# stresearch/xfr

Measured on AMD Instinct MI355X. Metric: triplet-contrastive-EBP saliency maps/sec, ResNet-101 224x224, higher is better.
Workload: dtype f32

## Files before the change

xfr_amd/csrc/conv_gemm.hip:

```cpp
#include <algorithm>
#include <atomic>
#include <mutex>
#include <vector>
#include "common.h"
#include <cstdio>
#include <cstdlib>

#include "conv_gemm_dev.h"
#include "conv_gemm_host.h"

std::atomic<long> g_conv_chain_launches[2];

namespace {

#ifndef XFR_MFM_WAVES
#define XFR_MFM_WAVES 6
#endif
#ifndef XFR_DUAL_WAVES
#define XFR_DUAL_WAVES 4
#endif
template <int TCO, int TM, int BK, int NST, int MODE, bool RELU, int CHAIN>
__global__ __launch_bounds__(NT, CHAIN == 0 ? 1 : (CHAIN == 1 ? 7 : (CHAIN == 4 ? XFR_DUAL_WAVES : XFR_MFM_WAVES))) void conv_gemm_kernel(const ConvParams p, const int n_co_tiles, const int n_m_tiles)
{
    constexpr bool ROW = TCO == 32;
// ... 722 lines not shown
        bool same = true;
        for (int i = 0; i < XFR_MAX_EW_STEPS && same; ++i) same = kChainSigs[sgi][i] == (i < n ? codes[i] : 0);
        if (same) return sgi;
    }
    return -1;
}
int conv_gemm_num_chain_sigs() { return kNumChainSigs; }

int conv_gemm_cannot_launch(const ConvParams& p)
{
    if (p.chain.n <= 0) return 0;
    ConvParams q = p;
    return plan_chain(q);
}
const char* conv_gemm_refusal(int why)
{
    switch (why) {
        case 0: return "the convolution launch was refused without a reason";
        case 1: return "a dual (W / relu(W)) convolution launch carries a fused chain without a compiled epilogue";
        case 3: return "lean probe-forward steps and the dual-accumulator launch (ConvParams::dualacc) only exist together, behind a compiled epilogue";
        case 2: return "a fused chain with a MaxFeatureMap step (pair maximum / fan-out VJP) has no compiled epilogue and the interpreter does not run those steps";
        default: return "unknown convolution launch refusal";
    }
}

void conv_gemm_chain_launch_counts(long* compiled, long* interpreted)
{
    if (compiled) *compiled = g_conv_chain_launches[0].load();
    if (interpreted) *interpreted = g_conv_chain_launches[1].load();
}

static int pick_cfg_impl(const ConvParams& p_in, bool allow_split)
{
    ConvParams p = p_in;
    if (p.dualacc) { p.nhalves = 2; p.dualacc = 0; const int c = pick_cfg_impl(p, false); return c == CFG_ROW32 ? CFG_K16 : c; }
    if (allow_split && p.split_ok && conv_gemm_split_wanted(p)) return CFG_BF16X6;
    {
        const int rem = p.CoutTot % 64;
#ifndef XFR_NO_ROW_TILE
        if (rem > 0 && rem <= 32 && p.tap_major != 2 && p.out_stride == 1 && p.CoutTot > 32 && p.M > 64) return CFG_ROW32;
#endif
    }
    if (ks_ok<8>(p)) {
        if (p.kh == 1 && (p.stride == 2 || p.out_stride == 2 || p.as_strided)) return CFG_KS_4_4;
        if ((p.kh > 1 && p.K >= 2048) || (p.kh == 1 && (p.K == 512 || p.K >= 2048))) return CFG_KS_4_4;
    }
    const long tiles = (long)((p.CoutTot + 63) / 64) * p.nhalves * ((p.M + 63) / 64);
    if (p.K >= 1024 && tiles <= 512 && (p.tap_major ? (p.Cin % 32 == 0) : true)) return CFG_K32;
    return CFG_K16;
}
int conv_gemm_pick_cfg(const ConvParams& p_in) { return pick_cfg_impl(p_in, true); }

namespace {
struct LogRec { void* stream; int cout, nhalves, K, M, kh, chain, cfg; };
std::mutex g_tune_mu;
std::atomic<int> g_tuning{0};
unsigned long long* g_stamps = nullptr;
int g_stamps_cap = 0;
int g_stamp_regions = 0, g_stamp_seq = 0;
unsigned long long* g_log = nullptr;
int g_log_cap = 0;
std::vector<LogRec> g_log_recs;
thread_local int g_last_cfg = 0;
constexpr size_t NO_LOG = (size_t)-1;

size_t tune_begin(ConvParams& p, hipStream_t s)
{
    p.stamps = nullptr;
    p.stamps_cap = 0;
    p.stamp_regions = 0;
    p.stamp_seq = 0;
    p.span = nullptr;
    size_t log_idx = NO_LOG;
    if (g_tuning.load(std::memory_order_relaxed)) {
        std::lock_guard<std::mutex> lk(g_tune_mu);
        p.stamps = g_stamps;
        p.stamps_cap = g_stamps_cap;
        p.stamp_regions = g_stamp_regions;
        p.stamp_seq = g_stamps ? g_stamp_seq++ : 0;
        if (g_log && (int)g_log_recs.size() < g_log_cap) {
            p.span = g_log + 8 * g_log_recs.size();
            log_idx = g_log_recs.size();
            g_log_recs.push_back(LogRec{(void*)s, p.CoutTot, p.dualacc ? 2 : p.nhalves, p.K, p.M, p.kh, p.chain.n, -1});
        }
    }
    return log_idx;
}
void tune_ran(size_t log_idx, int cfg)
{
    g_last_cfg = cfg;
    if (log_idx == NO_LOG) return;
    std::lock_guard<std::mutex> lk(g_tune_mu);
    if (log_idx < g_log_recs.size()) g_log_recs[log_idx].cfg = cfg;
}
int cfg_remap(int cfg)
{
    struct Remap { int v[32]; };
    static const Remap remap = [] {
        Remap r;
        for (int i = 0; i < 32; ++i) r.v[i] = i;
        if (const char* e = getenv("XFR_CFG_REMAP")) {
            int a = 0, b = 0, n = 0;
            while (sscanf(e, "%d:%d%n", &a, &b, &n) == 2) {
                if (a >= 0 && a < 32 && b >= 0 && b < 32) r.v[a] = b;
                e += n;
                if (*e == ',') ++e;
            }
        }
        return r;
    }();
    return (cfg >= 0 && cfg < 32) ? remap.v[cfg] : cfg;
}
}

void conv_gemm_set_stamps(unsigned long long* dev_ptr, int capacity_workgroups)
{
    std::lock_guard<std::mutex> lk(g_tune_mu);
    g_stamps = dev_ptr;
    g_stamps_cap = dev_ptr ? (capacity_workgroups < 0 ? -capacity_workgroups : capacity_workgroups) : 0;
    g_stamp_regions = (dev_ptr && capacity_workgroups < 0) ? (-capacity_workgroups) / 256 : 0;
    g_stamp_seq = 0;
    g_tuning.store((g_stamps || g_log) ? 1 : 0);
}

void conv_gemm_set_log(unsigned long long* log_dev, int capacity)
{
    std::lock_guard<std::mutex> lk(g_tune_mu);
    g_log = log_dev;
    g_log_cap = log_dev ? capacity : 0;
    g_log_recs.clear();
    g_tuning.store((g_stamps || g_log) ? 1 : 0);
}
int conv_gemm_dump_log(const char* path)
{
    std::lock_guard<std::mutex> lk(g_tune_mu);
    if (!g_log) return 0;
    const size_t n = g_log_recs.size();
    std::vector<unsigned long long> h(8 * n + 8);
    if (n && hipMemcpy(h.data(), g_log, 8 * n * sizeof(unsigned long long), hipMemcpyDeviceToHost) != hipSuccess) return -1;
    FILE* f = fopen(path, "w");
    if (!f) return -1;
    fprintf(f, "seq,stream,Cout,nhalves,K,M,kh,chain,cfg,start_10ns,end_10ns\n");
    for (size_t i = 0; i < n; ++i) {
        const LogRec& r = g_log_recs[i];
        fprintf(f, "%zu,%p,%d,%d,%d,%d,%d,%d,%d,%llu,%llu\n", i, r.stream, r.cout, r.nhalves, r.K, r.M, r.kh, r.chain, r.cfg, h[8 * i], *std::max_element(h.begin() + 8 * i + 1, h.begin() + 8 * i + 8));
    }
    fclose(f);
    return (int)n;
}
int conv_gemm_last_cfg() { return g_last_cfg; }

bool launch_conv_gemm(const ConvParams& p_in, hipStream_t s)
{
    ConvParams p = p_in;
    const size_t log_idx = tune_begin(p, s);
    int cfg = p.force_cfg > 0 ? p.force_cfg : cfg_remap(conv_gemm_pick_cfg(p));
    auto ran = [&](int eff, bool ok) { tune_ran(log_idx, eff); return ok; };
    if (cfg == CFG_BF16X6) {
        if (conv_gemm_launch_split(p, s)) return ran(CFG_BF16X6, true);
        cfg = pick_cfg_impl(p, false);
    }
    if (cfg == CFG_KS_8_3 && ks_ok<8>(p)) return ran(CFG_KS_8_3, launch_cfg_ks<8, 3>(p, s));
    if (cfg == CFG_KS_4_4 && ks_ok<4>(p)) return ran(CFG_KS_4_4, launch_cfg_ks<4, 4>(p, s));
    if (cfg == CFG_K32) return ran(CFG_K32, launch_cfg<64, 64, 32, 3>(p, s));
    if (cfg == CFG_ROW32) return ran(CFG_ROW32, launch_cfg<32, 128, 16, 3>(p, s));
    return ran(CFG_K16, launch_cfg<64, 64, 16, 3>(p, s));
}
```

xfr_amd/csrc/conv_gemm_host.h:

```cpp
#pragma once
#include <atomic>
#include "common.h"

extern std::atomic<long> g_conv_chain_launches[2];
int conv_gemm_num_cus();
int conv_gemm_plan_chain(ConvParams& q);
void conv_gemm_warn_interpreted(const ConvParams& q);
bool conv_gemm_launch_split(const ConvParams& p, hipStream_t s);
bool conv_gemm_split_wanted(const ConvParams& p);
```

xfr_amd/csrc/conv_gemm_split.hip:

```cpp
#include <algorithm>
#include <atomic>
#include <mutex>
#include <unordered_map>
#include <cstdio>
#include <cstdlib>
#include <type_traits>
#include "conv_gemm_dev.h"
#include "conv_gemm_host.h"

namespace {

typedef __bf16 v8bf __attribute__((ext_vector_type(8)));
typedef unsigned v4u __attribute__((ext_vector_type(4)));
constexpr int SP_T = 128, SP_BK = 16;
constexpr int SP_A_BYTES = 3 * 2 * SP_T * 16, SP_B_BYTES = 3 * 2 * SP_T * 16;
constexpr size_t SP_LDS = 3 * (size_t)(SP_A_BYTES + SP_B_BYTES);

typedef float v2f_t __attribute__((ext_vector_type(2)));
typedef __bf16 v2bf_t __attribute__((ext_vector_type(2)));
__device__ __forceinline__ unsigned cvt_pk_bf16(float lo, float hi)
{
    const v2f_t t = {lo, hi};
    return __builtin_bit_cast(unsigned, __builtin_convertvector(t, v2bf_t));
}
__device__ __forceinline__ void split_pair(float a, float b, unsigned& p0, unsigned& p1, unsigned& p2)
{
    p0 = cvt_pk_bf16(a, b);
    const float ra = a - __uint_as_float(p0 << 16), rb = b - __uint_as_float(p0 & 0xffff0000u);
    p1 = cvt_pk_bf16(ra, rb);
    const float sa = ra - __uint_as_float(p1 << 16), sb = rb - __uint_as_float(p1 & 0xffff0000u);
    p2 = cvt_pk_bf16(sa, sb);
}

constexpr int SPP_MAX_HALO = 64, SPP_MAX_TAPS = 25;

__host__ __device__ inline int spp_halo(const ConvParams& p) { return p.pad * p.W + p.pad; }
__host__ __device__ inline int spp_patch_len(const ConvParams& p) { return SP_T + 2 * spp_halo(p); }
inline size_t spp_lds_bytes(const ConvParams& p) { return (size_t)3 * SP_A_BYTES + (size_t)2 * 6 * (spp_patch_len(p) + 1) * 16; }

constexpr int NT8 = 512;

template <int N>
__device__ __forceinline__ void sp8_wait_barrier()
{
    asm volatile("s_waitcnt vmcnt(%0) lgkmcnt(0)\n\ts_barrier" ::"n"(N) : "memory");
}

template <bool RELU, int CHAIN, bool PATCH>
__global__ __launch_bounds__(NT8, 2) void conv_gemm_split_kernel(const ConvParams p, const uint16_t* __restrict__ ws0, const uint16_t* __restrict__ ws1,
                                                                  const int n_co_tiles, const int n_m_tiles)
{
    extern __shared__ __attribute__((aligned(16))) float smem[];
    unsigned char* lds = reinterpret_cast<unsigned char*>(smem);
    constexpr int NST = 3, D = NST - 1, XBASE = NST * SP_A_BYTES;
    const int tid = threadIdx.x, lane = tid & 63, wave8 = __builtin_amdgcn_readfirstlane(tid >> 6);
    const int wr4 = wave8 >> 1, wc = wave8 & 1;
    const int l31 = lane & 31, lhi = lane >> 5;
    const bool two_dma = wave8 < 4;
    if (wave8 < 4) stamp(p, wave8, lane, 0, 4);

    const int lid = xcd_remap(blockIdx.x, n_co_tiles * n_m_tiles);
    const int tile_m = lid / n_co_tiles;
    const int tile_co_all = lid - tile_m * n_co_tiles;
    const int n_co_half = n_co_tiles / p.nhalves;
    const int half = tile_co_all / n_co_half;
    const int tile_co = tile_co_all - half * n_co_half;
    const int co0 = tile_co * SP_T, m0 = tile_m * SP_T;
    const uint16_t* __restrict__ wsel = half ? ws1 : ws0;
    const float* __restrict__ bsel = half ? p.bias_pos : p.bias;
    float* __restrict__ osel = half ? p.out1 : p.out0;
    const int T = p.kh * p.kw, ncb = p.Cin / SP_BK, nk = p.K / SP_BK;
    const int halo = spp_halo(p), PL = spp_patch_len(p);
    const int PS = PATCH ? (PL + 1) * 16 : SP_T * 16;
    const int XB = 6 * PS;
    const unsigned chan_bytes = (unsigned)p.in_nb * p.H * p.W * 4u;
    const __amdgpu_buffer_rsrc_t rW = __builtin_amdgcn_make_buffer_rsrc((void*)wsel, 0, n_co_half * nk * SP_A_BYTES, 0x00020000);
    const __amdgpu_buffer_rsrc_t rIn = __builtin_amdgcn_make_buffer_rsrc((void*)p.in, 0, (int)p.in_bytes, 0x00020000);
    const unsigned lds_base = (unsigned)(size_t)(__attribute__((address_space(3))) unsigned char*)(lds);

    unsigned t_voff = OOB, t_lds = 0;
    bool t_ok = false;
    int base_m = 0;
    unsigned long long tapmask = 0ull;
    const int sm = tid & 127, skq = wave8 >> 1;
    if constexpr (PATCH) {
        const int kh_ = tid >= PL ? 1 : 0, q = tid - kh_ * PL;
        const long g = (long)m0 - halo + q;
        t_ok = tid < 2 * PL;
        const bool in_row = t_ok && g >= 0 && g < (long)p.in_nb * p.H * p.W;
        t_voff = in_row ? (unsigned)g * 4u + (unsigned)(kh_ * 8) * chan_bytes : OOB;
        t_lds = lds_base + XBASE + kh_ * PS + q * 16;
    } else {
        const int m = m0 + sm;
        const bool m_ok = m < p.M;
        const int mm = m_ok ? m : 0;
        const int ohw = p.OH * p.OW;
        const int n = mm / ohw;
        const int r = mm - n * ohw;
        const int oh = r / p.OW;
        const int ow = r - oh * p.OW;
        const int ih0 = oh * p.stride - p.pad, iw0 = ow * p.stride - p.pad - p.pad_dw;
        base_m = n * p.H * p.W + ih0 * p.W + iw0;
        if (m_ok) {
            unsigned long long vw = 0ull;
            for (int dw = 0; dw < p.kw; ++dw)
                if ((unsigned)(iw0 + dw) < (unsigned)p.W) vw |= 1ull << dw;
            for (int dh = 0; dh < p.kh; ++dh)
                if ((unsigned)(ih0 + dh) < (unsigned)p.H) tapmask |= vw << (dh * p.kw);
        }
        t_lds = lds_base + XBASE + ((skq >> 1) * SP_T + sm) * 16 + (skq & 1) * 8;
    }
    int c_pos[2] = {0, 0};
    unsigned c_mask[2] = {0u, 0u};
    if constexpr (PATCH) {
#pragma unroll
        for (int j = 0; j < 2; ++j) {
            const int c = wc * 64 + j * 32 + l31, m = m0 + c;
            c_pos[j] = c + halo;
            unsigned mk = 0u;
            if (m < p.M) {
                const int ohw = p.OH * p.OW;
                const int r = m % ohw;
                const int oh = r / p.OW, ow = r - oh * p.OW;
                for (int dh = 0; dh < p.kh; ++dh)
                    for (int dw = 0; dw < p.kw; ++dw)
                        if ((unsigned)(oh + dh - p.pad) < (unsigned)p.H && (unsigned)(ow + dw - p.pad) < (unsigned)p.W) mk |= 1u << (dh * p.kw + dw);
            }
            c_mask[j] = mk;
        }
    }
    const unsigned char* a_lane = lds + (lhi * SP_T + wr4 * 32 + l31) * 16;
    const unsigned char* b_plane = lds + XBASE + lhi * PS;

    v16f acc[2], pipe[2];
#pragma unroll
    for (int j = 0; j < 2; ++j)
#pragma unroll
        for (int r = 0; r < 16; ++r) { acc[j][r] = 0.f; pipe[j][r] = 0.f; }

    auto dma = [&](int kt, int stage, int ch) {
        __builtin_amdgcn_raw_ptr_buffer_load_lds(rW, (lptr_t)(lds + stage * SP_A_BYTES + ch * 1024), 16, (ch * 1024 + lane * 16) | (kt < nk ? 0u : OOB),
                                                 (tile_co * nk + kt) * SP_A_BYTES, 0, 0);
    };
    auto load_w = [&](int kt, int stage) {
        dma(kt, stage, wave8);
        if (two_dma) dma(kt, stage, 8 + wave8);
    };
    auto fold = [&](bool negated) {
        if (negated) { acc[0] -= pipe[0]; acc[1] -= pipe[1]; }
        else { acc[0] += pipe[0]; acc[1] += pipe[1]; }
    };
    auto mfmas = [&](const v8bf (&af)[3], const v8bf (&bf)[3][2], auto FIRST) {
        constexpr int TA[6] = {2, 1, 0, 1, 0, 0}, TB[6] = {0, 1, 2, 0, 1, 0};
        v16f zero;
#pragma unroll
        for (int r = 0; r < 16; ++r) zero[r] = 0.f;
#pragma unroll
        for (int t = 0; t < 6; ++t)
#pragma unroll
            for (int j = 0; j < 2; ++j)
                pipe[j] = __builtin_amdgcn_mfma_f32_32x32x16_bf16(af[TA[t]], bf[TB[t]][j], (t == 0 && decltype(FIRST)::value) ? zero : pipe[j], 0, 0, 0);
    };
    std::integral_constant<int, 0> S0; std::integral_constant<int, 1> S1; std::integral_constant<int, 2> S2;
    std::integral_constant<bool, true> first; std::integral_constant<bool, false> later;

    if constexpr (PATCH) {
        float xp[8];
        auto load_patch = [&](int cb) {
            const unsigned so = (unsigned)(cb * SP_BK) * chan_bytes;
#pragma unroll
            for (int i = 0; i < 8; ++i) xp[i] = __uint_as_float(__builtin_amdgcn_raw_buffer_load_b32(rIn, t_voff, so + (unsigned)i * chan_bytes, 0));
        };
        auto store_patch = [&](int buf, unsigned flip) {
            v4u q0, q1, q2;
#pragma unroll
            for (int i = 0; i < 4; ++i) {
                const float a = RELU ? fmaxf(xp[2 * i], 0.f) : xp[2 * i], b = RELU ? fmaxf(xp[2 * i + 1], 0.f) : xp[2 * i + 1];
                unsigned h0, h1, h2;
                split_pair(a, b, h0, h1, h2);
                q0[i] = h0 ^ flip; q1[i] = h1 ^ flip; q2[i] = h2 ^ flip;
            }
            if (t_ok) {
                const unsigned at = t_lds + buf * XB;
                asm volatile("ds_write_b128 %0, %1" :: "v"(at), "v"(q0));
                asm volatile("ds_write_b128 %0, %1" :: "v"(at + 2 * PS), "v"(q1));
                asm volatile("ds_write_b128 %0, %1" :: "v"(at + 4 * PS), "v"(q2));
            }
        };
        int tap = 0, cb = 0, buf = 0, shift = -halo, tdw = 0;
        bool xl_prev = false, xl_now = false;
        const bool mfma_first = wave8 < 4;
        auto load_part = [&](int kt, v8bf (&af)[3], v8bf (&bf)[3][2]) {
            const int st1 = (kt + 1) % 3, st3 = kt % 3;
            const bool more = cb + 1 < ncb;
            xl_now = false;
            if (more && tap == 2) store_patch(buf ^ 1, ((cb + 1) & 1) ? 0x80008000u : 0u);
            load_w(kt + 3, kt < 0 ? 2 : st3);
            if (more && tap == 0) { load_patch(cb + 1); xl_now = true; }
            const unsigned char* As = a_lane + (kt < 0 ? 0 : st1) * SP_A_BYTES;
#pragma unroll
            for (int pc = 0; pc < 3; ++pc) af[pc] = *(const v8bf*)(As + pc * 2 * SP_T * 16);
#pragma unroll
            for (int j = 0; j < 2; ++j) {
                const int pos = ((c_mask[j] >> tap) & 1u) ? c_pos[j] + shift : PL;
                const unsigned char* Bs = b_plane + buf * XB + pos * 16;
#pragma unroll
                for (int pc = 0; pc < 3; ++pc) bf[pc][j] = *(const v8bf*)(Bs + pc * 2 * PS);
            }
            tap += 1; tdw += 1; shift += 1;
            if (tdw == p.kw) { tdw = 0; shift += p.W - p.kw; }
            if (tap == T) { tap = 0; shift = -halo; cb += 1; buf ^= 1; }
        };
        auto end_step = [&]() {
            if (xl_now || xl_prev) { if (two_dma) sp8_wait_barrier<10>(); else sp8_wait_barrier<9>(); }
            else { if (two_dma) sp8_wait_barrier<2>(); else sp8_wait_barrier<1>(); }
            xl_prev = xl_now;
        };
        auto step = [&](int kt, v8bf (&caf)[3], v8bf (&cbf)[3][2], v8bf (&naf)[3], v8bf (&nbf)[3][2], auto FIRST) {
            if (mfma_first) mfmas(caf, cbf, FIRST);
            __builtin_amdgcn_sched_barrier(0);
            load_part(kt, naf, nbf);
            __builtin_amdgcn_sched_barrier(0);
            if (!mfma_first) mfmas(caf, cbf, FIRST);
            end_step();
        };
        if (tid < 12) {
            const v4u z = {0u, 0u, 0u, 0u};
            asm volatile("ds_write_b128 %0, %1" :: "v"(lds_base + XBASE + (tid / 6) * XB + (tid % 6) * PS + PL * 16), "v"(z));
        }
        load_w(0, 0);
        load_w(1, 1);
        load_patch(0);
        asm volatile("s_waitcnt vmcnt(0)" ::: "memory");
        store_patch(0, 0u);
        sp8_wait_barrier<0>();
        v8bf f0a[3], f0b[3][2], f1a[3], f1b[3][2];
        load_part(-1, f0a, f0b);
        end_step();
        if (wave8 < 4) stamp(p, wave8, lane, 1);
        int pass_in_blk = 0;
        bool neg = false;
        const int passes_per_blk = T / 3;
        auto pass_done = [&]() {
            fold(neg);
            if (++pass_in_blk == passes_per_blk) { pass_in_blk = 0; neg = !neg; }
        };
        for (int kt = 0; kt < nk; kt += 6) {
            step(kt, f0a, f0b, f1a, f1b, first);
            step(kt + 1, f1a, f1b, f0a, f0b, later);
            step(kt + 2, f0a, f0b, f1a, f1b, later);
            pass_done();
            step(kt + 3, f1a, f1b, f0a, f0b, first);
            step(kt + 4, f0a, f0b, f1a, f1b, later);
            step(kt + 5, f1a, f1b, f0a, f0b, later);
            pass_done();
        }
    } else {
        int ld_tap = 0, ld_ci0 = 0;
        unsigned ld_voff = (tapmask & 1ull) ? (unsigned)base_m * 4u : OOB;
        auto load_x = [&](int kt, float (&v)[4]) {
            const unsigned voff = ld_voff | (kt < nk ? 0u : OOB);
            const unsigned so = (unsigned)(ld_ci0 + skq * 4) * chan_bytes;
#pragma unroll
            for (int i = 0; i < 4; ++i) v[i] = __uint_as_float(__builtin_amdgcn_raw_buffer_load_b32(rIn, voff, so + (unsigned)i * chan_bytes, 0));
            ld_ci0 += SP_BK;
            if (ld_ci0 >= p.Cin) {
                ld_ci0 = 0;
                ld_tap += 1;
                const int dh = ld_tap / p.kw, dw = ld_tap - dh * p.kw;
                ld_voff = (ld_tap < p.kh * p.kw && ((tapmask >> ld_tap) & 1ull)) ? (unsigned)(base_m + dh * p.W + dw) * 4u : OOB;
            }
        };
        auto store_x = [&](const float (&v)[4], int stage, unsigned flip) {
            typedef unsigned v2u __attribute__((ext_vector_type(2)));
            v2u q0, q1, q2;
#pragma unroll
            for (int i = 0; i < 2; ++i) {
                const float a = RELU ? fmaxf(v[2 * i], 0.f) : v[2 * i], b = RELU ? fmaxf(v[2 * i + 1], 0.f) : v[2 * i + 1];
                unsigned h0, h1, h2;
                split_pair(a, b, h0, h1, h2);
                q0[i] = h0 ^ flip; q1[i] = h1 ^ flip; q2[i] = h2 ^ flip;
            }
            const unsigned at = t_lds + stage * XB;
            asm volatile("ds_write_b64 %0, %1" :: "v"(at), "v"(q0));
            asm volatile("ds_write_b64 %0, %1" :: "v"(at + 2 * PS), "v"(q1));
            asm volatile("ds_write_b64 %0, %1" :: "v"(at + 4 * PS), "v"(q2));
        };
        int wst = 0;
        auto step = [&](int kt, auto ST, float (&xcur)[4], float (&xnew)[4], unsigned flip, auto FIRST) {
            constexpr int st = decltype(ST)::value, st1 = (st + 1) % 3;
            const int stD = wst + D >= NST ? wst + D - NST : wst + D;
            load_w(kt + D, stD);
            load_x(kt + 3, xnew);
            const unsigned char* As = a_lane + wst * SP_A_BYTES;
            const unsigned char* Bs = b_plane + st * XB + (wc * 64 + l31) * 16;
            v8bf af[3], bf[3][2];
#pragma unroll
            for (int pc = 0; pc < 3; ++pc) {
                af[pc] = *(const v8bf*)(As + pc * 2 * SP_T * 16);
#pragma unroll
                for (int j = 0; j < 2; ++j) bf[pc][j] = *(const v8bf*)(Bs + pc * 2 * PS + j * 32 * 16);
            }
            mfmas(af, bf, FIRST);
            store_x(xcur, st1, flip);
            if (two_dma) sp8_wait_barrier<8 + 2 * (D - 1)>(); else sp8_wait_barrier<8 + (D - 1)>();
            wst = wst + 1 == NST ? 0 : wst + 1;
        };
        float x0[4], x1[4], x2[4];
        load_w(0, 0);
        load_x(0, x0);
        asm volatile("s_waitcnt vmcnt(0)" ::: "memory");
        store_x(x0, 0, 0u);
#pragma unroll
        for (int d = 1; d < D; ++d) load_w(d, d);
        load_x(1, x0);
        load_x(2, x1);
        if (two_dma) sp8_wait_barrier<8 + 2 * (D - 1)>(); else sp8_wait_barrier<8 + (D - 1)>();
        if (wave8 < 4) stamp(p, wave8, lane, 1);
        unsigned flip = 0u;
        for (int kt = 0; kt < nk; kt += 3) {
            const bool negated = flip != 0u;
            step(kt, S0, x0, x2, flip, first);
            step(kt + 1, S1, x1, x0, flip, later);
            flip ^= 0x80008000u;
            step(kt + 2, S2, x2, x1, flip, later);
            fold(negated);
        }
    }
    wait_vmcnt<0>();
    asm volatile("s_waitcnt lgkmcnt(0)" ::: "memory");
    if (wave8 < 4) { stamp(p, wave8, lane, 2); stamp(p, wave8, lane, 3); }

#pragma unroll 1
    for (int c = 0; c < 2; ++c) {
        v16f t = acc[0];
        const int wq = (wr4 & 1) * 2 + c;
        block_epilogue<CHAIN>(p, t, smem + (wave8 - wq) * (32 * 36), tid & 255, lane, wq, co0 + (wr4 >> 1) * 64, m0 + wc * 64, half, -1, 0, 1, osel, bsel, nullptr);
        acc[0] = acc[1];
    }
    if (wave8 < 4) stamp(p, wave8, lane, 4);
}

__global__ void split_pack_kernel(const float* __restrict__ w, uint16_t* __restrict__ planes, int K, int cout, int ldw, int taps)
{
    const long idx = (long)blockIdx.x * blockDim.x + threadIdx.x;
    if (idx >= (long)K * cout) return;
    const int k = (int)(idx / cout), co = (int)(idx - (long)k * cout);
    unsigned h[3];
    split_pair(w[(long)k * ldw + co], 0.f, h[0], h[1], h[2]);
    const int cin = K / taps, tap = k / cin, ci = k - tap * cin;
    const int rt = co / SP_T, r = co - rt * SP_T, kt = (ci / SP_BK) * taps + tap, kk = ci % SP_BK, nk = K / SP_BK;
#pragma unroll
    for (int q = 0; q < 3; ++q)
        planes[((((long)(rt * nk + kt) * 3 + q) * 2 + kk / 8) * SP_T + r) * 8 + kk % 8] = (uint16_t)(h[q] & 0xffffu);
}

struct SplitPack { uint16_t* planes; int K, cout, ldw, taps; };
static std::mutex g_split_mu;
static std::unordered_map<const float*, SplitPack> g_split;

bool split_can_run(const ConvParams& p)
{
    if (p.dualacc || p.out_stride != 1 || p.as_strided || p.co_pair > 0 || p.stride != 1) return false;
    if ((p.Cin % SP_BK) != 0 || (p.K % SP_BK) != 0 || (p.CoutTot % SP_T) != 0) return false;
    if (p.kh == 1 && p.kw == 1) return p.pad == 0;
    return p.tap_major == 1 && p.kh * p.kw <= 64;
}
struct SplitPolicy { int min_k1, min_k3, min_tiles; };
const SplitPolicy& split_policy()
{
    static const SplitPolicy pol = [] {
        SplitPolicy q{256, 1152, 128};
        if (const char* e = getenv("XFR_SPLIT_MIN_K1")) q.min_k1 = atoi(e);
        if (const char* e = getenv("XFR_SPLIT_MIN_K3")) q.min_k3 = atoi(e);
        if (const char* e = getenv("XFR_SPLIT_MIN_TILES")) q.min_tiles = atoi(e);
        return q;
    }();
    return pol;
}
bool split_layer_ok(const ConvParams& p)
{
    if (!split_can_run(p)) return false;
    if (p.OH * p.OW < 196) return false;
    return p.K >= (p.kh == 1 && p.kw == 1 ? split_policy().min_k1 : split_policy().min_k3);
}
bool split_grid_ok(const ConvParams& p)
{
    const long tiles = (long)(p.CoutTot / SP_T) * p.nhalves * ((p.M + SP_T - 1) / SP_T);
    return tiles >= split_policy().min_tiles;
}

static std::atomic<long> g_split_launches{0};

bool split_patch_ok(const ConvParams& p)
{
    const int T = p.kh * p.kw;
    if (T < 5 || T > SPP_MAX_TAPS || (T % 3) != 0 || p.stride != 1 || p.tap_major != 1) return false;
    if (p.OH != p.H || p.OW != p.W || 2 * p.pad != p.kh - 1 || 2 * p.pad != p.kw - 1 || p.pad_dw != 0) return false;
    static const bool off = getenv("XFR_SPLIT_NO_PATCH") != nullptr;
    return spp_halo(p) <= SPP_MAX_HALO && !off;
}

const uint16_t* split_planes(const float* w, int K, int cout, int ldw, int taps, hipStream_t s)
{
    std::lock_guard<std::mutex> lk(g_split_mu);
    auto it = g_split.find(w);
    if (it != g_split.end())
        return (it->second.K == K && it->second.cout == cout && it->second.ldw == ldw && it->second.taps == taps) ? it->second.planes : nullptr;
    SplitPack sp{nullptr, K, cout, ldw, taps};
    if (hipMalloc(&sp.planes, (size_t)K * cout * 3 * sizeof(uint16_t)) != hipSuccess) {
        (void)hipGetLastError();
        sp.planes = nullptr;
        g_split[w] = sp;
        return nullptr;
    }
    const long n = (long)K * cout;
    hipLaunchKernelGGL(split_pack_kernel, dim3((unsigned)((n + 255) / 256)), dim3(256), 0, s, w, sp.planes, K, cout, ldw, taps);
    if (hipStreamSynchronize(s) != hipSuccess) { (void)hipFree(sp.planes); return nullptr; }
    g_split[w] = sp;
    return sp.planes;
}

template <bool RELU, int CHAIN>
void launch_split_inst(const ConvParams& q, const uint16_t* w0, const uint16_t* w1, int n_co, int n_m, hipStream_t s, bool patch)
{
    static std::atomic<unsigned long long> done{0ull};
    int dev = 0;
    (void)hipGetDevice(&dev);
    const unsigned long long bit = 1ull << (dev & 63);
    constexpr int PATCH_LDS_MAX = 3 * SP_A_BYTES + 2 * 6 * (SP_T + 2 * SPP_MAX_HALO + 1) * 16;
    if (!(done.load(std::memory_order_relaxed) & bit)) {
        (void)hipFuncSetAttribute((const void*)conv_gemm_split_kernel<RELU, CHAIN, false>, hipFuncAttributeMaxDynamicSharedMemorySize, (int)SP_LDS);
        (void)hipFuncSetAttribute((const void*)conv_gemm_split_kernel<RELU, CHAIN, true>, hipFuncAttributeMaxDynamicSharedMemorySize, PATCH_LDS_MAX);
        done.fetch_or(bit);
    }
    const dim3 grid(n_co * n_m);
    if (patch) hipLaunchKernelGGL((conv_gemm_split_kernel<RELU, CHAIN, true>), grid, dim3(NT8), spp_lds_bytes(q), s, q, w0, w1, n_co, n_m);
    else hipLaunchKernelGGL((conv_gemm_split_kernel<RELU, CHAIN, false>), grid, dim3(NT8), SP_LDS, s, q, w0, w1, n_co, n_m);
}

bool launch_split(const ConvParams& p, hipStream_t s)
{
    if (p.force_cfg == CFG_BF16X6 ? !split_can_run(p) : !conv_gemm_split_wanted(p)) return false;
    if (p.chain.n > 0 && p.relu_in) return false;
    ConvParams q = p;
    q.tail_q = 0;
    q.tail_s = 1;
    int family = p.relu_in ? -1 : 0;
    if (q.chain.n > 0) {
        if (conv_gemm_plan_chain(q)) return false;
        if (q.chain_sig >= 0 && chain_sig_is_dual(q.chain_sig)) return false;
        family = q.chain_sig < 0 ? 2 : (chain_sig_is_mfm(q.chain_sig) ? 3 : 1);
    }
    const bool patch = split_patch_ok(p);
    const int taps = patch ? p.kh * p.kw : 1;
    const uint16_t* w0 = split_planes(p.w, p.K, p.CoutTot, p.ldw, taps, s);
    const uint16_t* w1 = p.nhalves == 2 ? split_planes(p.w_pos, p.K, p.CoutTot, p.ldw, taps, s) : nullptr;
    if (!w0 || (p.nhalves == 2 && !w1)) return false;
    g_split_launches++;
    if (q.chain.n > 0) {
        g_conv_chain_launches[q.chain_sig >= 0 ? 0 : 1]++;
        if (q.chain_sig < 0) conv_gemm_warn_interpreted(q);
    }
    const int n_co = (p.CoutTot / SP_T) * p.nhalves;
    const int n_m = (p.M + SP_T - 1) / SP_T;
    switch (family) {
        case -1: launch_split_inst<true, 0>(q, w0, w1, n_co, n_m, s, patch); break;
        case 0: launch_split_inst<false, 0>(q, w0, w1, n_co, n_m, s, patch); break;
        case 1: launch_split_inst<false, 1>(q, w0, w1, n_co, n_m, s, patch); break;
        case 2: launch_split_inst<false, 2>(q, w0, w1, n_co, n_m, s, patch); break;
        default: launch_split_inst<false, 3>(q, w0, w1, n_co, n_m, s, patch); break;
    }
    return true;
}

}

void conv_gemm_forget_split(const void* lo, size_t bytes)
{
    std::lock_guard<std::mutex> lk(g_split_mu);
    const char* a = static_cast<const char*>(lo);
    for (auto it = g_split.begin(); it != g_split.end();) {
        const char* w = reinterpret_cast<const char*>(it->first);
        if (w >= a && w < a + bytes) {
            if (it->second.planes) (void)hipFree(it->second.planes);
            it = g_split.erase(it);
        } else ++it;
    }
}
int conv_gemm_split_covers(const ConvParams& p) { return split_layer_ok(p) ? 1 : 0; }
bool conv_gemm_presplit(const ConvParams& p, const float* w, hipStream_t s) { return split_planes(w, p.K, p.CoutTot, p.ldw, split_patch_ok(p) ? p.kh * p.kw : 1, s) != nullptr; }
bool conv_gemm_split_wanted(const ConvParams& p) { return split_layer_ok(p) && (p.split_ok == 2 || split_grid_ok(p)); }
bool conv_gemm_launch_split(const ConvParams& p, hipStream_t s) { return launch_split(p, s); }
long conv_gemm_split_launches() { return g_split_launches.load(); }
```

xfr_amd/csrc/engine.hip:

```cpp
#include "engine_internal.h"

namespace xfr {

thread_local std::string g_err;

xfr_status fail(xfr_status st, const char* fmt, ...)
{
    char buf[1024];
    va_list ap;
    va_start(ap, fmt);
    vsnprintf(buf, sizeof(buf), fmt, ap);
    va_end(ap);
    g_err = buf;
    return st;
}

static xfr_status allocate(xfr_engine* e)
{
    xfr_status st = layout_arena(e);
    if (st != XFR_OK) return st;
    HIP_TRY(hipMalloc(&e->arena, e->arena_floats * sizeof(float)));
    st = layout_workspace(e);
    if (st != XFR_OK) return st;
    const size_t B = (size_t)e->max_batch;
// ... 824 lines not shown
{
    if (!e || !n_firings) return fail(XFR_INVALID_ARG, "null argument");
    *n_firings = e->last_trace_firings;
    return XFR_OK;
}

xfr_status xfr_engine_get_trace(xfr_engine* e, double* sums, int32_t* kinds, int32_t capacity)
{
    if (!e || !sums) return fail(XFR_INVALID_ARG, "null argument");
    const int nf = e->last_trace_firings, SB = e->last_trace_sb;
    if (capacity < nf * SB) return fail(XFR_INVALID_ARG, "trace needs %d doubles", nf * SB);
    HIP_TRY(hipSetDevice(e->device));
    HIP_TRY(hipDeviceSynchronize());
    HIP_TRY(hipMemcpy(sums, e->dbl_ws + 2 * e->max_batch, sizeof(double) * (size_t)nf * SB, hipMemcpyDeviceToHost));
    if (kinds) for (int i = 0; i < nf; ++i) kinds[i] = e->last_trace_kinds[i];
    return XFR_OK;
}

xfr_status xfr_debug_conv(const float* in_dev, const float* w_host, const float* bias_host, float* out_dev, int32_t cin, int32_t h,
                          int32_t w, int32_t nb, int32_t cout, int32_t kh, int32_t kw, int32_t stride, int32_t pad, int32_t relu_in,
                          int32_t cfg, int32_t reps, float* ms_out)
{
    if (!in_dev || !w_host || !out_dev || cin < 1 || cout < 1 || kh < 1 || kw < 1 || stride < 1 || reps < 1)
        return fail(XFR_INVALID_ARG, "xfr_debug_conv: bad arguments");
    const int khw = kh * kw, K = cin * khw;
    const int ldw = (int)align_up(cout, 128);
    const bool tap = khw > 1 && (cin % 16 == 0) && khw <= 64;
    const bool tap4 = khw > 1 && (cin == 3 || cin == 4) && khw <= 60;
    const int Kf = tap4 ? 4 * khw : K;
    std::vector<float> host(align_up(Kf, 32) * (size_t)ldw, 0.f);
    for (int co = 0; co < cout; ++co)
        for (int ci = 0; ci < cin; ++ci)
            for (int tp = 0; tp < khw; ++tp) {
                const size_t kk = tap4 ? (size_t)tp * 4 + ci : (tap ? (size_t)tp * cin + ci : (size_t)ci * khw + tp);
                host[kk * ldw + co] = w_host[((size_t)co * cin + ci) * khw + tp];
            }
    float *wd = nullptr, *bd = nullptr;
    HIP_TRY(hipMalloc(&wd, host.size() * sizeof(float)));
    HIP_TRY(hipMemcpy(wd, host.data(), host.size() * sizeof(float), hipMemcpyHostToDevice));
    if (bias_host) {
        HIP_TRY(hipMalloc(&bd, cout * sizeof(float)));
        HIP_TRY(hipMemcpy(bd, bias_host, cout * sizeof(float), hipMemcpyHostToDevice));
    }
    ConvParams p;
    memset(&p, 0, sizeof(p));
    p.in = in_dev; p.w = wd; p.bias = bd; p.out0 = out_dev;
    p.Cin = cin; p.H = h; p.W = w; p.NB = nb; p.in_nb = nb; p.out_nb = nb;
    p.kh = kh; p.kw = kw; p.stride = stride; p.pad = pad;
    p.OH = (h + 2 * pad - kh) / stride + 1; p.OW = (w + 2 * pad - kw) / stride + 1;
    p.K = Kf; p.K_logical = K; p.M = nb * p.OH * p.OW; p.CoutTot = cout; p.nhalves = 1; p.ldw = ldw;
    p.relu_in = relu_in; p.out_H = p.OH; p.out_W = p.OW; p.out_stride = 1;
    p.in_bytes = (unsigned)((size_t)cin * nb * h * w * sizeof(float));
    p.tap_major = tap4 ? 2 : (tap ? 1 : 0); p.force_cfg = cfg % 100;
    float* tws = nullptr;
    HIP_TRY(hipMalloc(&tws, XFR_TAIL_WS_BYTES + XFR_TAIL_MAX_TILES * sizeof(unsigned)));
    p.tail_ws = tws; p.tail_ws_bytes = XFR_TAIL_WS_BYTES;
    p.tail_cnt = reinterpret_cast<unsigned*>(reinterpret_cast<char*>(tws) + XFR_TAIL_WS_BYTES);
    HIP_TRY(hipMemset(p.tail_cnt, 0, XFR_TAIL_MAX_TILES * sizeof(unsigned)));
    p.tail_force = (cfg / 10000) % 100;
    const bool split = (cfg % 100) == CFG_BF16X6;
    hipEvent_t a, b;
    HIP_TRY(hipEventCreate(&a));
    HIP_TRY(hipEventCreate(&b));
    const int nstreams = std::max(1, std::min(4, cfg / 1000000));
    p.tail_force = (cfg / 10000) % 100;
    for (int r = 0; r < std::max(1, std::min(reps, 200)); ++r) launch_conv_gemm(p, 0);
    float ms = 0.f;
    if (nstreams == 1) {
        HIP_TRY(hipEventRecord(a, 0));
        for (int r = 0; r < reps; ++r) launch_conv_gemm(p, 0);
        HIP_TRY(hipEventRecord(b, 0));
        HIP_TRY(hipDeviceSynchronize());
        HIP_TRY(hipEventElapsedTime(&ms, a, b));
    } else {
        hipStream_t st[4];
        float* tw[4];
        ConvParams q[4];
        for (int i = 0; i < nstreams; ++i) {
            HIP_TRY(hipStreamCreateWithFlags(&st[i], hipStreamNonBlocking));
            HIP_TRY(hipMalloc(&tw[i], XFR_TAIL_WS_BYTES + XFR_TAIL_MAX_TILES * sizeof(unsigned)));
            q[i] = p;
            q[i].tail_ws = tw[i];
            q[i].tail_cnt = reinterpret_cast<unsigned*>(reinterpret_cast<char*>(tw[i]) + XFR_TAIL_WS_BYTES);
            HIP_TRY(hipMemset(q[i].tail_cnt, 0, XFR_TAIL_MAX_TILES * sizeof(unsigned)));
        }
        HIP_TRY(hipDeviceSynchronize());
        HIP_TRY(hipEventRecord(a, 0));
        for (int i = 0; i < nstreams; ++i) HIP_TRY(hipStreamWaitEvent(st[i], a, 0));
        for (int r = 0; r < reps; ++r)
            for (int i = 0; i < nstreams; ++i) launch_conv_gemm(q[i], st[i]);
        for (int i = 0; i < nstreams; ++i) {
            hipEvent_t e;
            HIP_TRY(hipEventCreateWithFlags(&e, hipEventDisableTiming));
            HIP_TRY(hipEventRecord(e, st[i]));
            HIP_TRY(hipStreamWaitEvent(0, e, 0));
            (void)hipEventDestroy(e);
        }
        HIP_TRY(hipEventRecord(b, 0));
        HIP_TRY(hipDeviceSynchronize());
        HIP_TRY(hipEventElapsedTime(&ms, a, b));
        ms /= nstreams;
        for (int i = 0; i < nstreams; ++i) { (void)hipStreamDestroy(st[i]); (void)hipFree(tw[i]); }
    }
    if (ms_out) *ms_out = ms / reps;
    (void)hipEventDestroy(a); (void)hipEventDestroy(b);
    if (split) conv_gemm_forget_split(wd, host.size() * sizeof(float));
    (void)hipFree(wd);
    (void)hipFree(tws);
    if (bd) (void)hipFree(bd);
    HIP_TRY(hipGetLastError());
    return XFR_OK;
}

xfr_status xfr_debug_conv_stamps(void* stamps_dev, int32_t capacity_workgroups)
{
    if (stamps_dev && (capacity_workgroups == 0 || (capacity_workgroups < 0 && -capacity_workgroups < 256)))
        return fail(XFR_INVALID_ARG, "xfr_debug_conv_stamps: capacity must be positive (or <= -256: sampled mode)");
    conv_gemm_set_stamps(reinterpret_cast<unsigned long long*>(stamps_dev), capacity_workgroups);
    return XFR_OK;
}

xfr_status xfr_debug_conv_log(void* log_dev, int32_t capacity, const char* dump_path)
{
    if (dump_path) {
        const int n = conv_gemm_dump_log(dump_path);
        if (n < 0) return fail(XFR_HIP_ERROR, "xfr_debug_conv_log: cannot write %s", dump_path);
    }
    conv_gemm_set_log(reinterpret_cast<unsigned long long*>(log_dev), capacity);
    return XFR_OK;
}

xfr_status xfr_engine_profile_csv(xfr_engine* e, const char* path)
{
    if (!e) return fail(XFR_INVALID_ARG, "null engine");
    e->profile_csv = path ? path : "";
    return XFR_OK;
}

xfr_status xfr_chain_epilogue_stats(int64_t* compiled_launches, int64_t* interpreted_launches, int32_t* n_signatures)
{
    long c = 0, i = 0;
    conv_gemm_chain_launch_counts(&c, &i);
    if (compiled_launches) *compiled_launches = c;
    if (interpreted_launches) *interpreted_launches = i;
    if (n_signatures) *n_signatures = conv_gemm_num_chain_sigs();
    return XFR_OK;
}

xfr_status xfr_engine_memory(xfr_engine* e, size_t* weight_bytes, size_t* workspace_bytes)
{
    if (!e) return fail(XFR_INVALID_ARG, "null engine");
    if (weight_bytes) *weight_bytes = e->arena_floats * sizeof(float);
    if (workspace_bytes) *workspace_bytes = e->ws_floats * sizeof(float) + e->idx_bytes;
    return XFR_OK;
}

xfr_status xfr_engine_set_profile(xfr_engine* e, int32_t enable)
{
    if (!e) return fail(XFR_INVALID_ARG, "null engine");
    e->profile_on = enable ? 1 : 0;
    return XFR_OK;
// ... 20 lines not shown
```

Measured before the change: 1551.

## Add split-K partitioning to the bf16x6 split conv kernel for small spatial layers

Lets the bf16x6 split GEMM kernel divide each output tile's K range across several workgroups. Each part writes its partial accumulators to a workspace slab, and the last part to arrive (tracked by an atomic counter) sums them and runs the epilogue. The minimum spatial size for using the split path drops from 196 to 49, and layers below 196 pixels may use up to 2 parts when the tile count is small, so 7x7/14x14 layers can fill more CUs. The cost is extra workspace traffic, atomics and a reduction pass. Logging also records the number of parts, and the debug bench now reuses its tail workspace across calls.

Result: faster. 1594 (median of 6 runs) (+2.8%).

```diff
diff --git a/xfr_amd/csrc/conv_gemm.hip b/xfr_amd/csrc/conv_gemm.hip
--- a/xfr_amd/csrc/conv_gemm.hip
+++ b/xfr_amd/csrc/conv_gemm.hip
@@ -798,7 +798,7 @@
 int conv_gemm_pick_cfg(const ConvParams& p_in) { return pick_cfg_impl(p_in, true); }
 
 namespace {
-struct LogRec { void* stream; int cout, nhalves, K, M, kh, chain, cfg; };
+struct LogRec { void* stream; int cout, nhalves, K, M, kh, chain, cfg, parts; };
 std::mutex g_tune_mu;
 std::atomic<int> g_tuning{0};
 unsigned long long* g_stamps = nullptr;
@@ -827,17 +827,17 @@
         if (g_log && (int)g_log_recs.size() < g_log_cap) {
             p.span = g_log + 8 * g_log_recs.size();
             log_idx = g_log_recs.size();
-            g_log_recs.push_back(LogRec{(void*)s, p.CoutTot, p.dualacc ? 2 : p.nhalves, p.K, p.M, p.kh, p.chain.n, -1});
+            g_log_recs.push_back(LogRec{(void*)s, p.CoutTot, p.dualacc ? 2 : p.nhalves, p.K, p.M, p.kh, p.chain.n, -1, 1});
         }
     }
     return log_idx;
 }
-void tune_ran(size_t log_idx, int cfg)
+void tune_ran(size_t log_idx, int cfg, int parts = 1)
 {
     g_last_cfg = cfg;
     if (log_idx == NO_LOG) return;
     std::lock_guard<std::mutex> lk(g_tune_mu);
-    if (log_idx < g_log_recs.size()) g_log_recs[log_idx].cfg = cfg;
+    if (log_idx < g_log_recs.size()) { g_log_recs[log_idx].cfg = cfg; g_log_recs[log_idx].parts = parts; }
 }
 int cfg_remap(int cfg)
 {
@@ -886,10 +886,10 @@
     if (n && hipMemcpy(h.data(), g_log, 8 * n * sizeof(unsigned long long), hipMemcpyDeviceToHost) != hipSuccess) return -1;
     FILE* f = fopen(path, "w");
     if (!f) return -1;
-    fprintf(f, "seq,stream,Cout,nhalves,K,M,kh,chain,cfg,start_10ns,end_10ns\n");
+    fprintf(f, "seq,stream,Cout,nhalves,K,M,kh,chain,cfg,start_10ns,end_10ns,parts\n");
     for (size_t i = 0; i < n; ++i) {
         const LogRec& r = g_log_recs[i];
-        fprintf(f, "%zu,%p,%d,%d,%d,%d,%d,%d,%d,%llu,%llu\n", i, r.stream, r.cout, r.nhalves, r.K, r.M, r.kh, r.chain, r.cfg, h[8 * i], *std::max_element(h.begin() + 8 * i + 1, h.begin() + 8 * i + 8));
+        fprintf(f, "%zu,%p,%d,%d,%d,%d,%d,%d,%d,%llu,%llu,%d\n", i, r.stream, r.cout, r.nhalves, r.K, r.M, r.kh, r.chain, r.cfg, h[8 * i], *std::max_element(h.begin() + 8 * i + 1, h.begin() + 8 * i + 8), r.parts);
     }
     fclose(f);
     return (int)n;
@@ -903,7 +903,7 @@
     int cfg = p.force_cfg > 0 ? p.force_cfg : cfg_remap(conv_gemm_pick_cfg(p));
     auto ran = [&](int eff, bool ok) { tune_ran(log_idx, eff); return ok; };
     if (cfg == CFG_BF16X6) {
-        if (conv_gemm_launch_split(p, s)) return ran(CFG_BF16X6, true);
+        if (conv_gemm_launch_split(p, s)) { tune_ran(log_idx, CFG_BF16X6, conv_gemm_split_last_parts()); return true; }
         cfg = pick_cfg_impl(p, false);
     }
     if (cfg == CFG_KS_8_3 && ks_ok<8>(p)) return ran(CFG_KS_8_3, launch_cfg_ks<8, 3>(p, s));
diff --git a/xfr_amd/csrc/conv_gemm_host.h b/xfr_amd/csrc/conv_gemm_host.h
--- a/xfr_amd/csrc/conv_gemm_host.h
+++ b/xfr_amd/csrc/conv_gemm_host.h
@@ -7,4 +7,5 @@
 int conv_gemm_plan_chain(ConvParams& q);
 void conv_gemm_warn_interpreted(const ConvParams& q);
 bool conv_gemm_launch_split(const ConvParams& p, hipStream_t s);
+int conv_gemm_split_last_parts();
 bool conv_gemm_split_wanted(const ConvParams& p);
diff --git a/xfr_amd/csrc/conv_gemm_split.hip b/xfr_amd/csrc/conv_gemm_split.hip
--- a/xfr_amd/csrc/conv_gemm_split.hip
+++ b/xfr_amd/csrc/conv_gemm_split.hip
@@ -59,7 +59,10 @@
     const bool two_dma = wave8 < 4;
     if (wave8 < 4) stamp(p, wave8, lane, 0, 4);
 
-    const int lid = xcd_remap(blockIdx.x, n_co_tiles * n_m_tiles);
+    const int nparts = p.tail_s > 1 ? p.tail_s : 1;
+    const int tile_lin = nparts > 1 ? (int)blockIdx.x / nparts : (int)blockIdx.x;
+    const int part = (int)blockIdx.x - tile_lin * nparts;
+    const int lid = xcd_remap(tile_lin, n_co_tiles * n_m_tiles);
     const int tile_m = lid / n_co_tiles;
     const int tile_co_all = lid - tile_m * n_co_tiles;
     const int n_co_half = n_co_tiles / p.nhalves;
@@ -70,6 +73,10 @@
     const float* __restrict__ bsel = half ? p.bias_pos : p.bias;
     float* __restrict__ osel = half ? p.out1 : p.out0;
     const int T = p.kh * p.kw, ncb = p.Cin / SP_BK, nk = p.K / SP_BK;
+    const int units = PATCH ? ncb : (nk + 2) / 3, ustep = PATCH ? T : 3;
+    const int ubase = units / nparts, urem = units - ubase * nparts;
+    const int u0 = part * ubase + min(part, urem), u1 = u0 + ubase + (part < urem ? 1 : 0);
+    const int k0 = u0 * ustep, k_end = min(u1 * ustep, nk);
     const int halo = spp_halo(p), PL = spp_patch_len(p);
     const int PS = PATCH ? (PL + 1) * 16 : SP_T * 16;
     const int XB = 6 * PS;
@@ -139,7 +146,7 @@
         for (int r = 0; r < 16; ++r) { acc[j][r] = 0.f; pipe[j][r] = 0.f; }
 
     auto dma = [&](int kt, int stage, int ch) {
-        __builtin_amdgcn_raw_ptr_buffer_load_lds(rW, (lptr_t)(lds + stage * SP_A_BYTES + ch * 1024), 16, (ch * 1024 + lane * 16) | (kt < nk ? 0u : OOB),
+        __builtin_amdgcn_raw_ptr_buffer_load_lds(rW, (lptr_t)(lds + stage * SP_A_BYTES + ch * 1024), 16, (ch * 1024 + lane * 16) | (kt < k_end ? 0u : OOB),
                                                  (tile_co * nk + kt) * SP_A_BYTES, 0, 0);
     };
     auto load_w = [&](int kt, int stage) {
@@ -187,15 +194,15 @@
                 asm volatile("ds_write_b128 %0, %1" :: "v"(at + 4 * PS), "v"(q2));
             }
         };
-        int tap = 0, cb = 0, buf = 0, shift = -halo, tdw = 0;
+        int tap = 0, cb = u0, buf = 0, shift = -halo, tdw = 0;
         bool xl_prev = false, xl_now = false;
         const bool mfma_first = wave8 < 4;
         auto load_part = [&](int kt, v8bf (&af)[3], v8bf (&bf)[3][2]) {
             const int st1 = (kt + 1) % 3, st3 = kt % 3;
-            const bool more = cb + 1 < ncb;
+            const bool more = cb + 1 < u1;
             xl_now = false;
             if (more && tap == 2) store_patch(buf ^ 1, ((cb + 1) & 1) ? 0x80008000u : 0u);
-            load_w(kt + 3, kt < 0 ? 2 : st3);
+            load_w(k0 + kt + 3, kt < 0 ? 2 : st3);
             if (more && tap == 0) { load_patch(cb + 1); xl_now = true; }
             const unsigned char* As = a_lane + (kt < 0 ? 0 : st1) * SP_A_BYTES;
 #pragma unroll
@@ -228,24 +235,28 @@
             const v4u z = {0u, 0u, 0u, 0u};
             asm volatile("ds_write_b128 %0, %1" :: "v"(lds_base + XBASE + (tid / 6) * XB + (tid % 6) * PS + PL * 16), "v"(z));
         }
-        load_w(0, 0);
-        load_w(1, 1);
-        load_patch(0);
+        if (u1 - u0 == 1) {
+            const v4u z = {0u, 0u, 0u, 0u};
+            for (int i = tid; i < 6 * (PL + 1); i += NT8) asm volatile("ds_write_b128 %0, %1" :: "v"(lds_base + XBASE + XB + i * 16), "v"(z));
+        }
+        load_w(k0, 0);
+        load_w(k0 + 1, 1);
+        load_patch(u0);
         asm volatile("s_waitcnt vmcnt(0)" ::: "memory");
-        store_patch(0, 0u);
+        store_patch(0, (u0 & 1) ? 0x80008000u : 0u);
         sp8_wait_barrier<0>();
         v8bf f0a[3], f0b[3][2], f1a[3], f1b[3][2];
         load_part(-1, f0a, f0b);
         end_step();
         if (wave8 < 4) stamp(p, wave8, lane, 1);
         int pass_in_blk = 0;
-        bool neg = false;
+        bool neg = (u0 & 1) != 0;
         const int passes_per_blk = T / 3;
         auto pass_done = [&]() {
             fold(neg);
             if (++pass_in_blk == passes_per_blk) { pass_in_blk = 0; neg = !neg; }
         };
-        for (int kt = 0; kt < nk; kt += 6) {
+        for (int kt = 0; kt < k_end - k0; kt += 6) {
             step(kt, f0a, f0b, f1a, f1b, first);
             step(kt + 1, f1a, f1b, f0a, f0b, later);
             step(kt + 2, f0a, f0b, f1a, f1b, later);
@@ -256,10 +267,10 @@
             pass_done();
         }
     } else {
-        int ld_tap = 0, ld_ci0 = 0;
-        unsigned ld_voff = (tapmask & 1ull) ? (unsigned)base_m * 4u : OOB;
+        int ld_tap = (k0 * SP_BK) / p.Cin, ld_ci0 = k0 * SP_BK - ld_tap * p.Cin;
+        unsigned ld_voff = (ld_tap < T && ((tapmask >> ld_tap) & 1ull)) ? (unsigned)(base_m + (ld_tap / p.kw) * p.W + ld_tap % p.kw) * 4u : OOB;
         auto load_x = [&](int kt, float (&v)[4]) {
-            const unsigned voff = ld_voff | (kt < nk ? 0u : OOB);
+            const unsigned voff = ld_voff | (kt < k_end ? 0u : OOB);
             const unsigned so = (unsigned)(ld_ci0 + skq * 4) * chan_bytes;
 #pragma unroll
             for (int i = 0; i < 4; ++i) v[i] = __uint_as_float(__builtin_amdgcn_raw_buffer_load_b32(rIn, voff, so + (unsigned)i * chan_bytes, 0));
@@ -307,18 +318,18 @@
             wst = wst + 1 == NST ? 0 : wst + 1;
         };
         float x0[4], x1[4], x2[4];
-        load_w(0, 0);
-        load_x(0, x0);
+        unsigned flip = (u0 & 1) ? 0x80008000u : 0u;
+        load_w(k0, 0);
+        load_x(k0, x0);
         asm volatile("s_waitcnt vmcnt(0)" ::: "memory");
-        store_x(x0, 0, 0u);
-#pragma unroll
-        for (int d = 1; d < D; ++d) load_w(d, d);
-        load_x(1, x0);
-        load_x(2, x1);
+        store_x(x0, 0, flip);
+#pragma unroll
+        for (int d = 1; d < D; ++d) load_w(k0 + d, d);
+        load_x(k0 + 1, x0);
+        load_x(k0 + 2, x1);
         if (two_dma) sp8_wait_barrier<8 + 2 * (D - 1)>(); else sp8_wait_barrier<8 + (D - 1)>();
         if (wave8 < 4) stamp(p, wave8, lane, 1);
-        unsigned flip = 0u;
-        for (int kt = 0; kt < nk; kt += 3) {
+        for (int kt = k0; kt < k_end; kt += 3) {
             const bool negated = flip != 0u;
             step(kt, S0, x0, x2, flip, first);
             step(kt + 1, S1, x1, x0, flip, later);
@@ -329,7 +340,45 @@
     }
     wait_vmcnt<0>();
     asm volatile("s_waitcnt lgkmcnt(0)" ::: "memory");
-    if (wave8 < 4) { stamp(p, wave8, lane, 2); stamp(p, wave8, lane, 3); }
+    if (wave8 < 4) stamp(p, wave8, lane, 2);
+
+    if (nparts > 1) {
+        constexpr int TILE_FLOATS = SP_T * SP_T;
+        float* __restrict__ slab = p.tail_ws + ((long)tile_lin * nparts + part) * TILE_FLOATS + tid;
+#pragma unroll
+        for (int j = 0; j < 2; ++j)
+#pragma unroll
+            for (int r = 0; r < 16; ++r) __hip_atomic_store(slab + (j * 16 + r) * NT8, acc[j][r], __ATOMIC_RELAXED, __HIP_MEMORY_SCOPE_AGENT);
+        wait_vmcnt<0>();
+        __syncthreads();
+        int* flag = reinterpret_cast<int*>(smem);
+        if (tid == 0) {
+            const unsigned old = atomicAdd(p.tail_cnt + tile_lin, 1u);
+            const int last = (old == (unsigned)(nparts - 1));
+            if (last) atomicExch(p.tail_cnt + tile_lin, 0u);
+            *flag = last;
+        }
+        __syncthreads();
+        const int last_part = *flag;
+        __syncthreads();
+        if (!last_part) {
+            if (wave8 < 4) { stamp(p, wave8, lane, 3); stamp(p, wave8, lane, 4); }
+            return;
+        }
+        const float* __restrict__ src = p.tail_ws + (long)tile_lin * nparts * TILE_FLOATS + tid;
+#pragma unroll
+        for (int j = 0; j < 2; ++j)
+#pragma unroll
+            for (int r = 0; r < 16; ++r) acc[j][r] = 0.f;
+        for (int q = 0; q < nparts; ++q, src += TILE_FLOATS) {
+            float v[32];
+#pragma unroll
+            for (int r = 0; r < 32; ++r) v[r] = __hip_atomic_load(src + r * NT8, __ATOMIC_RELAXED, __HIP_MEMORY_SCOPE_AGENT);
+#pragma unroll
+            for (int r = 0; r < 32; ++r) acc[r >> 4][r & 15] += v[r];
+        }
+    }
+    if (wave8 < 4) stamp(p, wave8, lane, 3);
 
 #pragma unroll 1
     for (int c = 0; c < 2; ++c) {
@@ -359,39 +408,6 @@
 static std::mutex g_split_mu;
 static std::unordered_map<const float*, SplitPack> g_split;
 
-bool split_can_run(const ConvParams& p)
-{
-    if (p.dualacc || p.out_stride != 1 || p.as_strided || p.co_pair > 0 || p.stride != 1) return false;
-    if ((p.Cin % SP_BK) != 0 || (p.K % SP_BK) != 0 || (p.CoutTot % SP_T) != 0) return false;
-    if (p.kh == 1 && p.kw == 1) return p.pad == 0;
-    return p.tap_major == 1 && p.kh * p.kw <= 64;
-}
-struct SplitPolicy { int min_k1, min_k3, min_tiles; };
-const SplitPolicy& split_policy()
-{
-    static const SplitPolicy pol = [] {
-        SplitPolicy q{256, 1152, 128};
-        if (const char* e = getenv("XFR_SPLIT_MIN_K1")) q.min_k1 = atoi(e);
-        if (const char* e = getenv("XFR_SPLIT_MIN_K3")) q.min_k3 = atoi(e);
-        if (const char* e = getenv("XFR_SPLIT_MIN_TILES")) q.min_tiles = atoi(e);
-        return q;
-    }();
-    return pol;
-}
-bool split_layer_ok(const ConvParams& p)
-{
-    if (!split_can_run(p)) return false;
-    if (p.OH * p.OW < 196) return false;
-    return p.K >= (p.kh == 1 && p.kw == 1 ? split_policy().min_k1 : split_policy().min_k3);
-}
-bool split_grid_ok(const ConvParams& p)
-{
-    const long tiles = (long)(p.CoutTot / SP_T) * p.nhalves * ((p.M + SP_T - 1) / SP_T);
-    return tiles >= split_policy().min_tiles;
-}
-
-static std::atomic<long> g_split_launches{0};
-
 bool split_patch_ok(const ConvParams& p)
 {
     const int T = p.kh * p.kw;
@@ -400,6 +416,63 @@
     static const bool off = getenv("XFR_SPLIT_NO_PATCH") != nullptr;
     return spp_halo(p) <= SPP_MAX_HALO && !off;
 }
+
+bool split_can_run(const ConvParams& p)
+{
+    if (p.dualacc || p.out_stride != 1 || p.as_strided || p.co_pair > 0 || p.stride != 1) return false;
+    if ((p.Cin % SP_BK) != 0 || (p.K % SP_BK) != 0 || (p.CoutTot % SP_T) != 0) return false;
+    if (p.kh == 1 && p.kw == 1) return p.pad == 0;
+    return p.tap_major == 1 && p.kh * p.kw <= 64;
+}
+struct SplitPolicy { int min_k1, min_k3, min_tiles, min_hw, max_parts, min_steps, min_cb, parts_below_hw; };
+const SplitPolicy& split_policy()
+{
+    static const SplitPolicy pol = [] {
+        SplitPolicy q{256, 1152, 128, 49, 2, 32, 4, 196};
+        if (const char* e = getenv("XFR_SPLIT_MIN_K1")) q.min_k1 = atoi(e);
+        if (const char* e = getenv("XFR_SPLIT_MIN_K3")) q.min_k3 = atoi(e);
+        if (const char* e = getenv("XFR_SPLIT_MIN_TILES")) q.min_tiles = atoi(e);
+        if (const char* e = getenv("XFR_SPLIT_MIN_HW")) q.min_hw = atoi(e);
+        if (const char* e = getenv("XFR_SPLIT_MAX_PARTS")) q.max_parts = atoi(e);
+        if (const char* e = getenv("XFR_SPLIT_MIN_STEPS")) q.min_steps = atoi(e);
+        if (const char* e = getenv("XFR_SPLIT_MIN_CB")) q.min_cb = atoi(e);
+        if (const char* e = getenv("XFR_SPLIT_PARTS_BELOW_HW")) q.parts_below_hw = atoi(e);
+        return q;
+    }();
+    return pol;
+}
+bool split_layer_ok(const ConvParams& p)
+{
+    if (!split_can_run(p)) return false;
+    if (p.OH * p.OW < split_policy().min_hw) return false;
+    return p.K >= (p.kh == 1 && p.kw == 1 ? split_policy().min_k1 : split_policy().min_k3);
+}
+int split_pick_parts(const ConvParams& p)
+{
+    if (!p.tail_ws || !p.tail_cnt || p.tail_force == 1) return 1;
+    const long tiles = (long)(p.CoutTot / SP_T) * p.nhalves * ((p.M + SP_T - 1) / SP_T);
+    if (tiles > XFR_TAIL_MAX_TILES) return 1;
+    const bool patch = split_patch_ok(p);
+    const int nk = p.K / SP_BK, units = patch ? p.Cin / SP_BK : (nk + 2) / 3;
+    const long fit = std::min<long>(units, (long)(p.tail_ws_bytes / ((size_t)SP_T * SP_T * sizeof(float))) / tiles);
+    if (p.tail_force >= 2) return (int)std::max<long>(1, std::min<long>(p.tail_force, fit));
+    const SplitPolicy& pol = split_policy();
+    if (p.OH * p.OW >= pol.parts_below_hw) return 1;
+    const long resident = patch ? 256 : 512;
+    const int min_units = patch ? pol.min_cb : (pol.min_steps + 2) / 3;
+    int S = 1;
+    for (int s = 2; s <= pol.max_parts && s <= fit; ++s)
+        if (tiles * s <= resident && units / s >= min_units) S = s;
+    return S;
+}
+bool split_grid_ok(const ConvParams& p)
+{
+    const long tiles = (long)(p.CoutTot / SP_T) * p.nhalves * ((p.M + SP_T - 1) / SP_T);
+    return tiles * split_pick_parts(p) >= split_policy().min_tiles;
+}
+
+static std::atomic<long> g_split_launches{0};
+static thread_local int g_split_last_parts = 1;
 
 const uint16_t* split_planes(const float* w, int K, int cout, int ldw, int taps, hipStream_t s)
 {
@@ -434,7 +507,7 @@
         (void)hipFuncSetAttribute((const void*)conv_gemm_split_kernel<RELU, CHAIN, true>, hipFuncAttributeMaxDynamicSharedMemorySize, PATCH_LDS_MAX);
         done.fetch_or(bit);
     }
-    const dim3 grid(n_co * n_m);
+    const dim3 grid(n_co * n_m * (q.tail_s > 1 ? q.tail_s : 1));
     if (patch) hipLaunchKernelGGL((conv_gemm_split_kernel<RELU, CHAIN, true>), grid, dim3(NT8), spp_lds_bytes(q), s, q, w0, w1, n_co, n_m);
     else hipLaunchKernelGGL((conv_gemm_split_kernel<RELU, CHAIN, false>), grid, dim3(NT8), SP_LDS, s, q, w0, w1, n_co, n_m);
 }
@@ -445,7 +518,7 @@
     if (p.chain.n > 0 && p.relu_in) return false;
     ConvParams q = p;
     q.tail_q = 0;
-    q.tail_s = 1;
+    q.tail_s = split_pick_parts(p);
     int family = p.relu_in ? -1 : 0;
     if (q.chain.n > 0) {
         if (conv_gemm_plan_chain(q)) return false;
@@ -458,6 +531,7 @@
     const uint16_t* w1 = p.nhalves == 2 ? split_planes(p.w_pos, p.K, p.CoutTot, p.ldw, taps, s) : nullptr;
     if (!w0 || (p.nhalves == 2 && !w1)) return false;
     g_split_launches++;
+    g_split_last_parts = q.tail_s;
     if (q.chain.n > 0) {
         g_conv_chain_launches[q.chain_sig >= 0 ? 0 : 1]++;
         if (q.chain_sig < 0) conv_gemm_warn_interpreted(q);
@@ -493,3 +567,4 @@
 bool conv_gemm_split_wanted(const ConvParams& p) { return split_layer_ok(p) && (p.split_ok == 2 || split_grid_ok(p)); }
 bool conv_gemm_launch_split(const ConvParams& p, hipStream_t s) { return launch_split(p, s); }
 long conv_gemm_split_launches() { return g_split_launches.load(); }
+int conv_gemm_split_last_parts() { return g_split_last_parts; }
diff --git a/xfr_amd/csrc/engine.hip b/xfr_amd/csrc/engine.hip
--- a/xfr_amd/csrc/engine.hip
+++ b/xfr_amd/csrc/engine.hip
@@ -900,11 +900,13 @@
     p.relu_in = relu_in; p.out_H = p.OH; p.out_W = p.OW; p.out_stride = 1;
     p.in_bytes = (unsigned)((size_t)cin * nb * h * w * sizeof(float));
     p.tap_major = tap4 ? 2 : (tap ? 1 : 0); p.force_cfg = cfg % 100;
-    float* tws = nullptr;
-    HIP_TRY(hipMalloc(&tws, XFR_TAIL_WS_BYTES + XFR_TAIL_MAX_TILES * sizeof(unsigned)));
+    static float* tws = nullptr;
+    if (!tws) {
+        HIP_TRY(hipMalloc(&tws, XFR_TAIL_WS_BYTES + XFR_TAIL_MAX_TILES * sizeof(unsigned)));
+        HIP_TRY(hipMemset(reinterpret_cast<char*>(tws) + XFR_TAIL_WS_BYTES, 0, XFR_TAIL_MAX_TILES * sizeof(unsigned)));
+    }
     p.tail_ws = tws; p.tail_ws_bytes = XFR_TAIL_WS_BYTES;
     p.tail_cnt = reinterpret_cast<unsigned*>(reinterpret_cast<char*>(tws) + XFR_TAIL_WS_BYTES);
-    HIP_TRY(hipMemset(p.tail_cnt, 0, XFR_TAIL_MAX_TILES * sizeof(unsigned)));
     p.tail_force = (cfg / 10000) % 100;
     const bool split = (cfg % 100) == CFG_BF16X6;
     hipEvent_t a, b;
@@ -954,7 +956,6 @@
     (void)hipEventDestroy(a); (void)hipEventDestroy(b);
     if (split) conv_gemm_forget_split(wd, host.size() * sizeof(float));
     (void)hipFree(wd);
-    (void)hipFree(tws);
     if (bd) (void)hipFree(bd);
     HIP_TRY(hipGetLastError());
     return XFR_OK;
```
